# sigp/lighthouse

Hardware: AMD Instinct MI355X
Metric: bls_sig_sets_verified_per_sec (higher is better)
Workload: dtype u64; 1 GPU; c2_64k_attestation_sets_plus_c3_registry_root; n_sets_per_gpu=65536, set_mix=75% k=1 unagg, 25% aggregates k=512, n_validators=1048576, parallelism=single, full=False

## Files before the change

### include/m3x_consensus.h

```cpp
#ifndef M3X_CONSENSUS_H
#define M3X_CONSENSUS_H
#include <stdint.h>
#include <stddef.h>

#ifdef __cplusplus
extern "C" {
#endif

typedef struct m3x_ctx m3x_ctx;

#define M3X_OK 0
#define M3X_ERR_HIP -1
#define M3X_ERR_ARG -2
#define M3X_ERR_NOMEM -3
#define M3X_ERR_ENCODING -4

int32_t m3x_ctx_create(m3x_ctx **out, int32_t device);
void m3x_ctx_destroy(m3x_ctx *ctx);
int32_t m3x_abi_version(void);

int32_t m3x_timing_enable(m3x_ctx *ctx, int32_t on);
int32_t m3x_kernel_ms(m3x_ctx *ctx, int32_t kernel_id, double *ms,
                      uint64_t *launches);

// ... 6 lines not shown
int32_t m3x_h2d(m3x_ctx *ctx, void *dst_dev, const void *src_host,
                uint64_t bytes);
int32_t m3x_d2h(m3x_ctx *ctx, void *dst_host, const void *src_dev,
                uint64_t bytes);


int32_t m3x_merkleize_validators(m3x_ctx *ctx, const uint8_t *ssz, uint64_t n,
                                 uint8_t out_root[32]);
int32_t m3x_merkleize_validators_dev(m3x_ctx *ctx, const void *ssz_dev,
                                     uint64_t n, uint8_t out_root[32]);

int32_t m3x_merkleize_chunks(m3x_ctx *ctx, const uint8_t *chunks,
                             uint64_t n_chunks, uint32_t depth,
                             int64_t mix_len, uint8_t out_root[32]);
int32_t m3x_merkleize_chunks_dev(m3x_ctx *ctx, const void *chunks_dev,
                                 uint64_t n_chunks, uint32_t depth,
                                 int64_t mix_len, uint8_t out_root[32]);

int32_t m3x_validator_subtree_root_dev(m3x_ctx *ctx, const void *ssz_dev,
                                       uint64_t n, uint32_t depth,
                                       uint8_t out_root[32]);

typedef struct m3x_registry_cache m3x_registry_cache;

int32_t m3x_registry_cache_create(m3x_ctx *ctx, const uint8_t *ssz,
                                  uint64_t n, m3x_registry_cache **out);
void m3x_registry_cache_destroy(m3x_registry_cache *cache);
int32_t m3x_registry_cache_root(m3x_ctx *ctx, m3x_registry_cache *cache,
                                uint8_t out_root[32]);
int32_t m3x_registry_cache_update(m3x_ctx *ctx, m3x_registry_cache *cache,
                                  const uint64_t *indices,
                                  const uint8_t *recs , uint64_t m,
                                  uint8_t out_root[32]);

int32_t m3x_merkleize_batch(m3x_ctx *ctx, const uint8_t *chunks,
                            const uint32_t *offsets, uint64_t n_elems,
                            uint8_t *out_roots);

int32_t m3x_shuffle_list(m3x_ctx *ctx, uint32_t *indices, uint64_t list_size,
                         uint32_t rounds, const uint8_t seed[32],
                         int32_t forwards);
int32_t m3x_shuffle_list_dev(m3x_ctx *ctx, void *indices_dev,
                             uint64_t list_size, uint32_t rounds,
                             const uint8_t seed[32], int32_t forwards);


int32_t m3x_bls_expand_test(m3x_ctx *ctx, const uint8_t *msg,
                            uint32_t msg_len, const uint8_t *dst,
                            uint32_t dst_len, uint32_t len_in_bytes,
                            uint8_t *out);
int32_t m3x_bls_h2c_test(m3x_ctx *ctx, const uint8_t *msg, uint32_t msg_len,
                         const uint8_t *dst, uint32_t dst_len,
                         uint8_t out_uncomp[192], uint8_t out_uniform[256]);

int32_t m3x_bls_sig_sum_test(m3x_ctx *ctx, const uint8_t *sigs ,
                             const uint64_t *rands , uint64_t n,
                             int32_t use_msm, uint8_t out_uncomp[192]);

int32_t m3x_bls_pk_decompress(m3x_ctx *ctx, const uint8_t *comp ,
                              uint64_t n, uint8_t *uncomp ,
                              int32_t *status );

int32_t m3x_bls_sig_aggregate(m3x_ctx *ctx, const uint8_t *sigs ,
                              uint64_t n, uint8_t out_sig[96]);

int32_t m3x_bls_verify_sets(m3x_ctx *ctx, const uint8_t *msgs,
                            const uint8_t *sigs, const uint8_t *pks,
                            const uint32_t *pk_offsets, const uint64_t *rands,
                            uint64_t n);
int32_t m3x_bls_verify_sets_dev(m3x_ctx *ctx, const void *msgs_dev,
                                const void *sigs_dev, const void *pks_dev,
                                const void *pk_offsets_dev,
                                const void *rands_dev, uint64_t n);

int32_t m3x_bls_verify_each(m3x_ctx *ctx, const uint8_t *msgs,
                            const uint8_t *sigs, const uint8_t *pks,
                            const uint32_t *pk_offsets, uint64_t n,
                            int32_t *verdicts );
int32_t m3x_bls_verify_each_dev(m3x_ctx *ctx, const void *msgs_dev,
                                const void *sigs_dev, const void *pks_dev,
                                const void *pk_offsets_dev, uint64_t n,
                                void *verdicts_dev );

typedef struct m3x_kzg m3x_kzg;

int32_t m3x_kzg_create(m3x_ctx *ctx, const uint8_t g2_tau[96],
                       m3x_kzg **out);
void m3x_kzg_destroy(m3x_kzg *kzg);

int32_t m3x_kzg_verify_proof(m3x_ctx *ctx, m3x_kzg *kzg, const uint8_t c[48],
                             const uint8_t z[32], const uint8_t y[32],
                             const uint8_t proof[48]);
int32_t m3x_kzg_verify_proof_batch(m3x_ctx *ctx, m3x_kzg *kzg,
                                   const uint8_t *cs, const uint8_t *zs,
                                   const uint8_t *ys, const uint8_t *proofs,
                                   uint64_t n);
int32_t m3x_kzg_verify_blob_proof_batch(m3x_ctx *ctx, m3x_kzg *kzg,
                                        const uint8_t *blobs,
                                        const uint8_t *cs,
                                        const uint8_t *proofs, uint64_t n);
int32_t m3x_kzg_verify_blob_proof_batch_dev(m3x_ctx *ctx, m3x_kzg *kzg,
                                            const void *blobs_dev,
                                            const void *cs_dev,
                                            const void *proofs_dev,
                                            uint64_t n);

// ... 97 lines not shown
```

### lighthouse_amd/_native.py

```python
import ctypes
import os
import threading
from pathlib import Path

_PKG = Path(__file__).resolve().parent
_LIB_PATH = _PKG / "libm3x_consensus.so"

_lib = None
_load_error = None


def _bind(lib):
    lib.m3x_abi_version.restype = ctypes.c_int32
    lib.m3x_ctx_create.argtypes = [ctypes.POINTER(ctypes.c_void_p), ctypes.c_int32]
    lib.m3x_ctx_create.restype = ctypes.c_int32
    lib.m3x_ctx_destroy.argtypes = [ctypes.c_void_p]
    lib.m3x_dev_alloc.argtypes = [
        ctypes.c_void_p,
        ctypes.c_uint64,
        ctypes.POINTER(ctypes.c_void_p),
    ]
    lib.m3x_dev_alloc.restype = ctypes.c_int32
    lib.m3x_dev_free.argtypes = [ctypes.c_void_p, ctypes.c_void_p]
    lib.m3x_dev_free.restype = ctypes.c_int32
# ... 97 lines not shown
            ],
        ),
        (
            "m3x_merkleize_batch",
            [
                ctypes.c_void_p,
                ctypes.c_char_p,
                ctypes.POINTER(ctypes.c_uint32),
                ctypes.c_uint64,
                ctypes.c_char_p,
            ],
        ),
        (
            "m3x_kernel_ms",
            [
                ctypes.c_void_p,
                ctypes.c_int32,
                ctypes.POINTER(ctypes.c_double),
                ctypes.POINTER(ctypes.c_uint64),
            ],
        ),
        (
            "m3x_finalize_root",
            [
                ctypes.c_void_p,
                ctypes.c_char_p,
                ctypes.c_uint32,
                ctypes.c_uint32,
                ctypes.c_int64,
                ctypes.c_char_p,
            ],
        ),
        (
            "m3x_bls_expand_test",
            [
                ctypes.c_void_p,
                ctypes.c_char_p,
                ctypes.c_uint32,
                ctypes.c_char_p,
                ctypes.c_uint32,
                ctypes.c_uint32,
                ctypes.c_char_p,
            ],
        ),
        (
            "m3x_bls_h2c_test",
            [
                ctypes.c_void_p,
                ctypes.c_char_p,
                ctypes.c_uint32,
                ctypes.c_char_p,
                ctypes.c_uint32,
                ctypes.c_char_p,
                ctypes.c_char_p,
            ],
        ),
        (
            "m3x_bls_sig_sum_test",
            [
                ctypes.c_void_p,
                ctypes.c_char_p,
                ctypes.POINTER(ctypes.c_uint64),
                ctypes.c_uint64,
                ctypes.c_int32,
                ctypes.c_char_p,
            ],
        ),
        (
            "m3x_bls_pk_decompress",
            [
                ctypes.c_void_p,
                ctypes.c_char_p,
                ctypes.c_uint64,
                ctypes.c_char_p,
                ctypes.POINTER(ctypes.c_int32),
            ],
        ),
        (
            "m3x_bls_verify_sets",
            [
                ctypes.c_void_p,
                ctypes.c_char_p,
                ctypes.c_char_p,
                ctypes.c_char_p,
                ctypes.POINTER(ctypes.c_uint32),
                ctypes.POINTER(ctypes.c_uint64),
                ctypes.c_uint64,
            ],
        ),
        (
            "m3x_bls_verify_sets_dev",
            [
                ctypes.c_void_p,
                ctypes.c_void_p,
                ctypes.c_void_p,
                ctypes.c_void_p,
                ctypes.c_void_p,
                ctypes.c_void_p,
                ctypes.c_uint64,
            ],
        ),
        (
            "m3x_bls_verify_each",
            [
                ctypes.c_void_p,
                ctypes.c_char_p,
# ... 322 lines not shown
```

### lighthouse_amd/csrc/bls_device.hh

```
#pragma once
#include <hip/hip_runtime.h>
#include <stdint.h>
#include "bls_consts.h"
#include "sha256.hh"

namespace m3xb {

struct fp {
  uint64_t v[6];
};

struct fp2 {
  fp c0, c1;
};

struct g1a {
  fp x, y;
  int inf;
};
struct g1j {
  fp x, y, z;
};
struct g2a {
  fp2 x, y;
  int inf;
};
struct g2j {
  fp2 x, y, z;
};


__device__ __forceinline__ bool fp_ge_p(const uint64_t t[6]) {
#pragma unroll
  for (int i = 5; i >= 0; i--) {
    if (t[i] > BLS_P[i]) return true;
    if (t[i] < BLS_P[i]) return false;
  }
  return true;
}

__device__ __forceinline__ void fp_sub_p(uint64_t t[6]) {
  unsigned __int128 bw = 0;
#pragma unroll
  for (int i = 0; i < 6; i++) {
    unsigned __int128 x = (unsigned __int128)t[i] - BLS_P[i] - (uint64_t)bw;
    t[i] = (uint64_t)x;
    bw = (x >> 64) & 1;
  }
}

__device__ __forceinline__ void fp_add(fp &r, const fp &a, const fp &b) {
  unsigned __int128 c = 0;
  uint64_t t[6];
#pragma unroll
  for (int i = 0; i < 6; i++) {
    c += (unsigned __int128)a.v[i] + b.v[i];
// ... 180 lines not shown
__device__ __forceinline__ void fp_from_std(fp &r, const uint64_t std[6]) {
  fp s, r2;
#pragma unroll
  for (int i = 0; i < 6; i++) {
    s.v[i] = std[i];
    r2.v[i] = BLS_R2[i];
  }
  fp_mul(r, s, r2);
}

#define FP_LOAD_C(dst, NAME)                                                   \
  do {                                                                         \
    uint64_t _std[6] = {NAME[0], NAME[1], NAME[2], NAME[3], NAME[4], NAME[5]}; \
    fp_from_std(dst, _std);                                                    \
  } while (0)

__device__ __forceinline__ void fp_to_std(uint64_t std[6], const fp &a) {
  fp one_std;
#pragma unroll
  for (int i = 0; i < 6; i++) one_std.v[i] = (i == 0) ? 1ull : 0ull;
  fp t;
  fp_mul(t, a, one_std);
#pragma unroll
  for (int i = 0; i < 6; i++) std[i] = t.v[i];
}

__device__ inline void fp_pow_limbs(fp &r, const fp &a, const uint64_t *e,
                                    int n) {
  fp acc;
  fp_one(acc);
  bool started = false;
  for (int i = n - 1; i >= 0; i--) {
    for (int b = 63; b >= 0; b--) {
      if (started) fp_sqr(acc, acc);
      if ((e[i] >> b) & 1) {
        if (started)
          fp_mul(acc, acc, a);
        else {
          acc = a;
          started = true;
        }
      }
    }
  }
  r = acc;
}

__device__ inline void fp_inv(fp &r, const fp &a) {
  uint64_t e[6] = {BLS_P[0] - 2, BLS_P[1], BLS_P[2],
                   BLS_P[3], BLS_P[4], BLS_P[5]};
  fp_pow_limbs(r, a, e, 6);
}

__device__ inline bool fp_sqrt(fp &r, const fp &a) {
  uint64_t t[6] = {BLS_P[0] + 1, BLS_P[1], BLS_P[2],
                   BLS_P[3], BLS_P[4], BLS_P[5]};
  uint64_t e[6];
#pragma unroll
  for (int i = 0; i < 6; i++)
    e[i] = (t[i] >> 2) | (i < 5 ? (t[i + 1] << 62) : 0);
  fp s, s2;
  fp_pow_limbs(s, a, e, 6);
  fp_sqr(s2, s);
  if (!fp_eq(s2, a)) return false;
  r = s;
  return true;
}

__device__ inline bool fp_sqrt_ui(fp &s, fp &u, const fp &a) {
  uint64_t t[6] = {BLS_P[0] - 3, BLS_P[1], BLS_P[2],
                   BLS_P[3], BLS_P[4], BLS_P[5]};
  uint64_t e[6];
#pragma unroll
  for (int i = 0; i < 6; i++)
    e[i] = (t[i] >> 2) | (i < 5 ? (t[i + 1] << 62) : 0);
  fp_pow_limbs(u, a, e, 6);
  fp_mul(s, u, a);
  fp s2;
  fp_sqr(s2, s);
  return fp_eq(s2, a);
}

__device__ inline bool fp_gt_half(const fp &a) {
  uint64_t s[6];
  fp_to_std(s, a);
  uint64_t pm1[6] = {BLS_P[0] - 1, BLS_P[1], BLS_P[2],
                     BLS_P[3], BLS_P[4], BLS_P[5]};
  uint64_t h[6];
#pragma unroll
  for (int i = 0; i < 6; i++)
    h[i] = (pm1[i] >> 1) | (i < 5 ? (pm1[i + 1] << 63) : 0);
#pragma unroll
  for (int i = 5; i >= 0; i--) {
    if (s[i] > h[i]) return true;
    if (s[i] < h[i]) return false;
  }
  return false;
}

__device__ inline bool fp_is_odd_std(const fp &a) {
  uint64_t s[6];
  fp_to_std(s, a);
  return s[0] & 1;
}

__device__ inline bool fp_from_be48(fp &r, const uint8_t *b) {
  uint64_t s[6];
#pragma unroll
  for (int i = 0; i < 6; i++) {
    uint64_t w = 0;
#pragma unroll
    for (int j = 0; j < 8; j++) w = (w << 8) | b[8 * i + j];
    s[5 - i] = w;
  }
  if (fp_ge_p(s)) return false;
  fp_from_std(r, s);
  return true;
}

__device__ inline void fp_to_be48(const fp &a, uint8_t *b) {
  uint64_t s[6];
  fp_to_std(s, a);
#pragma unroll
  for (int i = 0; i < 6; i++)
#pragma unroll
    for (int j = 0; j < 8; j++)
      b[8 * i + j] = (uint8_t)(s[5 - i] >> (56 - 8 * j));
}

// ... 35 lines not shown
__device__ __forceinline__ void fp2_mul(fp2 &r, const fp2 &a, const fp2 &b) {
  fp t0, t1, s0, s1, m;
  fp_mul(t0, a.c0, b.c0);
  fp_mul(t1, a.c1, b.c1);
  fp_add(s0, a.c0, a.c1);
  fp_add(s1, b.c0, b.c1);
  fp_mul(m, s0, s1);
  fp_sub(m, m, t0);
  fp_sub(m, m, t1);
  fp_sub(r.c0, t0, t1);
  r.c1 = m;
}

__device__ __forceinline__ void fp2_sqr(fp2 &r, const fp2 &a) {
  fp s, d, m;
  fp_add(s, a.c0, a.c1);
  fp_sub(d, a.c0, a.c1);
  fp_mul(m, a.c0, a.c1);
  fp_mul(s, s, d);
  fp_add(r.c1, m, m);
  r.c0 = s;
}

__device__ __forceinline__ void fp2_mul_fp(fp2 &r, const fp2 &a, const fp &k) {
  fp_mul(r.c0, a.c0, k);
  fp_mul(r.c1, a.c1, k);
}

__device__ __forceinline__ void fp2_mul_small(fp2 &r, const fp2 &a, int k) {
  fp2 acc = a;
  for (int i = 1; i < k; i++) fp2_add(acc, acc, a);
  r = acc;
}

__device__ inline void fp2_inv(fp2 &r, const fp2 &a) {
  fp n, t0, t1;
  fp_sqr(t0, a.c0);
  fp_sqr(t1, a.c1);
  fp_add(n, t0, t1);
  fp_inv(n, n);
  fp_mul(r.c0, a.c0, n);
  fp_mul(t0, a.c1, n);
  fp_neg(r.c1, t0);
}

__device__ __forceinline__ void fp2_mul_xi(fp2 &r, const fp2 &a) {
  fp t0, t1;
  fp_sub(t0, a.c0, a.c1);
  fp_add(t1, a.c0, a.c1);
  r.c0 = t0;
  r.c1 = t1;
}

__device__ inline bool fp2_sqrt(fp2 &r, const fp2 &a) {
  if (fp2_is_zero(a)) {
    fp2_zero(r);
    return true;
  }
  if (fp_is_zero(a.c1)) {
    fp s;
    if (fp_sqrt(s, a.c0)) {
      r.c0 = s;
      fp_zero(r.c1);
      return true;
    }
    fp na;
    fp_neg(na, a.c0);
    if (!fp_sqrt(s, na)) return false;
    fp_zero(r.c0);
    r.c1 = s;
    return true;
  }
  fp n, s, d, x0, x1, t, u, inv2;
  fp_sqr(n, a.c0);
  fp_sqr(t, a.c1);
  fp_add(n, n, t);
  if (!fp_sqrt(s, n)) return false;
  FP_LOAD_C(inv2, FP_TWO_INV);
  fp_add(d, a.c0, s);
  fp_mul(d, d, inv2);
  if (!fp_sqrt_ui(x0, u, d)) {
    fp_sub(d, a.c0, s);
    fp_mul(d, d, inv2);
    if (!fp_sqrt_ui(x0, u, d)) return false;
  }
  fp_mul(x1, a.c1, u);
  fp_mul(x1, x1, inv2);
  fp2 cand, sq;
  cand.c0 = x0;
  cand.c1 = x1;
  fp2_sqr(sq, cand);
  if (!fp2_eq(sq, a)) return false;
  r = cand;
  return true;
}

__device__ inline bool fp2_gt_half_lex(const fp2 &y) {
  if (!fp_is_zero(y.c1)) return fp_gt_half(y.c1);
  if (!fp_is_zero(y.c0)) return fp_gt_half(y.c0);
  return false;
}

__device__ inline int fp2_sgn0(const fp2 &x) {
  int s0 = fp_is_odd_std(x.c0) ? 1 : 0;
  int z0 = fp_is_zero(x.c0) ? 1 : 0;
  int s1 = fp_is_odd_std(x.c1) ? 1 : 0;
  return s0 | (z0 & s1);
}

#define FP2_LOAD_C(dst, NAME)                                                  \
  do {                                                                         \
    FP_LOAD_C((dst).c0, NAME##_C0);                                            \
    FP_LOAD_C((dst).c1, NAME##_C1);                                            \
  } while (0)


__device__ __forceinline__ bool g1j_is_inf(const g1j &p) {
  return fp_is_zero(p.z);
}

__device__ __forceinline__ void g1j_set_inf(g1j &p) {
  fp_zero(p.x);
  fp_zero(p.y);
  fp_zero(p.z);
}

__device__ inline void g1j_from_aff(g1j &r, const g1a &a) {
  if (a.inf) {
    g1j_set_inf(r);
    return;
  }
  r.x = a.x;
  r.y = a.y;
  fp_one(r.z);
}

__device__ inline void g1j_to_aff(g1a &r, const g1j &p) {
  if (g1j_is_inf(p)) {
    r.inf = 1;
    fp_zero(r.x);
    fp_zero(r.y);
    return;
  }
// ... 1290 lines not shown
  for (int i = 0; i < dst_len; i++) cur[33 + i] = (uint8_t)DSTs[i];
  cur[33 + dst_len] = (uint8_t)dst_len;
  uint8_t bi[32];
  m3x::sha256_bytes(cur, 33 + dst_len + 1, bi);
  for (int i = 0; i < 32; i++) out[i] = bi[i];
  for (int blk = 2; blk <= 8; blk++) {
    for (int j = 0; j < 32; j++) cur[j] = b0[j] ^ bi[j];
    cur[32] = (uint8_t)blk;
    m3x::sha256_bytes(cur, 33 + dst_len + 1, bi);
    for (int j = 0; j < 32; j++) {
      bi[j] = bi[j];
      out[32 * (blk - 1) + j] = bi[j];
    }
  }
}

__device__ inline void expand_message_xmd_gen(const uint8_t *msg,
                                              uint32_t msg_len,
                                              const uint8_t *dst,
                                              uint32_t dst_len,
                                              uint32_t len_in_bytes,
                                              uint8_t *out) {
  uint32_t ell = (len_in_bytes + 31) / 32;
  uint8_t buf[64 + 544 + 2 + 1 + 255 + 1];
  uint32_t off = 0;
  for (int i = 0; i < 64; i++) buf[off++] = 0;
  for (uint32_t i = 0; i < msg_len; i++) buf[off++] = msg[i];
  buf[off++] = (uint8_t)(len_in_bytes >> 8);
  buf[off++] = (uint8_t)len_in_bytes;
  buf[off++] = 0;
  for (uint32_t i = 0; i < dst_len; i++) buf[off++] = dst[i];
  buf[off++] = (uint8_t)dst_len;
  uint8_t b0[32];
  m3x::sha256_bytes(buf, off, b0);
  uint8_t cur[32 + 1 + 255 + 1];
  for (int i = 0; i < 32; i++) cur[i] = b0[i];
  cur[32] = 1;
  for (uint32_t i = 0; i < dst_len; i++) cur[33 + i] = dst[i];
  cur[33 + dst_len] = (uint8_t)dst_len;
  uint8_t bi[32];
  m3x::sha256_bytes(cur, 33 + dst_len + 1, bi);
  uint32_t copied = len_in_bytes < 32 ? len_in_bytes : 32;
  for (uint32_t i = 0; i < copied; i++) out[i] = bi[i];
  for (uint32_t blk = 2; blk <= ell; blk++) {
    for (int j = 0; j < 32; j++) cur[j] = b0[j] ^ bi[j];
    cur[32] = (uint8_t)blk;
    m3x::sha256_bytes(cur, 33 + dst_len + 1, bi);
    uint32_t base = 32 * (blk - 1);
    uint32_t nc = len_in_bytes - base < 32 ? len_in_bytes - base : 32;
    for (uint32_t i = 0; i < nc; i++) out[base + i] = bi[i];
  }
}

__device__ inline void sswu_g2_tail(g2a &out, const fp2 &u, const fp2 &zu2,
                                    const fp2 &inv_tv_p1, bool tv_zero) {
  fp2 A, B;
  FP2_LOAD_C(A, SSWU_A);
  FP2_LOAD_C(B, SSWU_B);
  fp2 x1, gx1, y1, x, y, t;
  if (tv_zero) {
    FP2_LOAD_C(x1, SSWU_B_DIV_ZA);
  } else {
    fp2 nb_over_a;
    FP2_LOAD_C(nb_over_a, SSWU_NB_DIV_A);
    fp2_mul(x1, nb_over_a, inv_tv_p1);
  }
  fp2_sqr(gx1, x1);
  fp2_mul(gx1, gx1, x1);
  fp2_mul(t, A, x1);
  fp2_add(gx1, gx1, t);
  fp2_add(gx1, gx1, B);
  if (fp2_sqrt(y1, gx1)) {
    x = x1;
    y = y1;
  } else {
    fp2 x2, gx2;
    fp2_mul(x2, zu2, x1);
    fp2_sqr(gx2, x2);
    fp2_mul(gx2, gx2, x2);
    fp2_mul(t, A, x2);
    fp2_add(gx2, gx2, t);
    fp2_add(gx2, gx2, B);
    fp2_sqrt(y1, gx2);
    x = x2;
    y = y1;
  }
  if (fp2_sgn0(u) != fp2_sgn0(y)) fp2_neg(y, y);
  out.x = x;
  out.y = y;
  out.inf = 0;
}

__device__ inline void sswu_g2(g2a &out, const fp2 &u) {
  fp2 Z, zu2, tv, inv_tv;
  FP2_LOAD_C(Z, SSWU_Z);
  fp2_sqr(zu2, u);
  fp2_mul(zu2, zu2, Z);
  fp2_sqr(tv, zu2);
  fp2_add(tv, tv, zu2);
  bool tz = fp2_is_zero(tv);
  fp2_zero(inv_tv);
  if (!tz) {
    fp2 one;
    fp2_inv(inv_tv, tv);
    fp2_one(one);
    fp2_add(inv_tv, one, inv_tv);
  }
  sswu_g2_tail(out, u, zu2, inv_tv, tz);
}

__device__ inline void sswu_g2_dual(g2a out[2], const fp2 u[2]) {
  fp2 Z, zu2[2], tv[2];
  FP2_LOAD_C(Z, SSWU_Z);
  bool tz[2];
  for (int i = 0; i < 2; i++) {
    fp2_sqr(zu2[i], u[i]);
    fp2_mul(zu2[i], zu2[i], Z);
    fp2_sqr(tv[i], zu2[i]);
    fp2_add(tv[i], tv[i], zu2[i]);
    tz[i] = fp2_is_zero(tv[i]);
  }
  fp2 inv[2], one;
  fp2_one(one);
  if (!tz[0] && !tz[1]) {
    fp2 prod, pinv;
    fp2_mul(prod, tv[0], tv[1]);
    fp2_inv(pinv, prod);
    fp2_mul(inv[0], pinv, tv[1]);
    fp2_mul(inv[1], pinv, tv[0]);
  } else {
    for (int i = 0; i < 2; i++) {
      fp2_zero(inv[i]);
      if (!tz[i]) fp2_inv(inv[i], tv[i]);
    }
  }
  for (int i = 0; i < 2; i++) {
    fp2_add(inv[i], inv[i], one);
    sswu_g2_tail(out[i], u[i], zu2[i], inv[i], tz[i]);
  }
}

__device__ inline void iso_map_g2_j(g2j &out, const g2a &in) {
  fp2 k[4], xn, xd, yn, yd;
  FP2_LOAD_C(k[0], ISO_XNUM0);
  FP2_LOAD_C(k[1], ISO_XNUM1);
  FP2_LOAD_C(k[2], ISO_XNUM2);
  FP2_LOAD_C(k[3], ISO_XNUM3);
  xn = k[3];
  for (int i = 2; i >= 0; i--) {
    fp2_mul(xn, xn, in.x);
    fp2_add(xn, xn, k[i]);
  }
  FP2_LOAD_C(k[0], ISO_XDEN0);
  FP2_LOAD_C(k[1], ISO_XDEN1);
  FP2_LOAD_C(k[2], ISO_XDEN2);
  xd = k[2];
  for (int i = 1; i >= 0; i--) {
    fp2_mul(xd, xd, in.x);
    fp2_add(xd, xd, k[i]);
  }
  FP2_LOAD_C(k[0], ISO_YNUM0);
  FP2_LOAD_C(k[1], ISO_YNUM1);
  FP2_LOAD_C(k[2], ISO_YNUM2);
  FP2_LOAD_C(k[3], ISO_YNUM3);
  yn = k[3];
  for (int i = 2; i >= 0; i--) {
    fp2_mul(yn, yn, in.x);
    fp2_add(yn, yn, k[i]);
  }
  FP2_LOAD_C(k[0], ISO_YDEN0);
  FP2_LOAD_C(k[1], ISO_YDEN1);
  FP2_LOAD_C(k[2], ISO_YDEN2);
  FP2_LOAD_C(k[3], ISO_YDEN3);
  yd = k[3];
  for (int i = 2; i >= 0; i--) {
    fp2_mul(yd, yd, in.x);
    fp2_add(yd, yd, k[i]);
  }
  fp2 yd2, xd2, xd3, t;
  fp2_sqr(yd2, yd);
  fp2_sqr(xd2, xd);
  fp2_mul(xd3, xd2, xd);
  fp2_mul(out.z, xd, yd);
  fp2_mul(t, xn, xd);
  fp2_mul(out.x, t, yd2);
  fp2_mul(t, yd2, xd3);
  fp2_mul(t, t, yn);
  fp2_mul(out.y, t, in.y);
}

__device__ inline void g2j_neg(g2j &r, const g2j &p) {
  r.x = p.x;
// ... 1 lines not shown
  r.z = p.z;
}

__device__ inline void psi_g2j(g2j &r, const g2j &p) {
  fp2 cx, cy, t;
  FP2_LOAD_C(cx, PSI_CX);
  FP2_LOAD_C(cy, PSI_CY);
  fp2_conj(t, p.x);
  fp2_mul(r.x, t, cx);
  fp2_conj(t, p.y);
  fp2_mul(r.y, t, cy);
  fp2_conj(r.z, p.z);
}

__device__ inline void g2j_mul_u64_j(g2j &r, const g2j &base, uint64_t k) {
  g2j acc;
  g2j_set_inf(acc);
  for (int b = 63; b >= 0; b--) {
    g2j_dbl(acc, acc);
    if ((k >> b) & 1) g2j_add(acc, acc, base);
  }
  r = acc;
}

__device__ inline void clear_cofactor_g2j(g2j &out, const g2j &p) {
  g2j xp, xxp, acc, tmp, d;
  g2j_mul_u64_j(xp, p, BLS_X_ABS);
  g2j_neg(xp, xp);
  g2j_mul_u64_j(xxp, xp, BLS_X_ABS);
  g2j_neg(xxp, xxp);
  acc = xxp;
  g2j_neg(tmp, xp);
  g2j_add(acc, acc, tmp);
  g2j_neg(tmp, p);
  g2j_add(acc, acc, tmp);
  d = xp;
  g2j_neg(tmp, p);
  g2j_add(d, d, tmp);
  psi_g2j(tmp, d);
  g2j_add(acc, acc, tmp);
  g2j_dbl(tmp, p);
  psi_g2j(tmp, tmp);
  psi_g2j(tmp, tmp);
  g2j_add(acc, acc, tmp);
  out = acc;
}

__device__ inline void h2c_g2_from_uniform(g2j &r, const uint8_t uni[256]) {
  fp2 u[2];
  h2f_from_be64(u[0].c0, uni);
  h2f_from_be64(u[0].c1, uni + 64);
  h2f_from_be64(u[1].c0, uni + 128);
  h2f_from_be64(u[1].c1, uni + 192);
  g2a qp[2];
  sswu_g2_dual(qp, u);
  g2j s, t;
  iso_map_g2_j(s, qp[0]);
  iso_map_g2_j(t, qp[1]);
  g2j_add(s, s, t);
  clear_cofactor_g2j(r, s);
}

__device__ inline void h2c_g2(g2j &r, const uint8_t *msg) {
  uint8_t uni[256];
  expand_message_xmd32(msg, uni);
  h2c_g2_from_uniform(r, uni);
}

__device__ inline void g2_to_uncomp_dev(const g2a &p, uint8_t *out) {
  fp_to_be48(p.x.c1, out);
  fp_to_be48(p.x.c0, out + 48);
  fp_to_be48(p.y.c1, out + 96);
  fp_to_be48(p.y.c0, out + 144);
}

__device__ inline void g1_gen(g1a &g) {
  FP_LOAD_C(g.x, BLS_G1X);
  FP_LOAD_C(g.y, BLS_G1Y);
  g.inf = 0;
}


template <typename T, int W, typename Op>
__device__ __forceinline__ void block_tree_reduce(T *lds, int t, Op op) {
  __syncthreads();
  for (int s = W / 2; s > 0; s >>= 1) {
    if (t < s) {
      T r;
      op(r, lds[t], lds[t + s]);
      lds[t] = r;
    }
    __syncthreads();
  }
}

struct g1j_add_op {
  __device__ __forceinline__ void operator()(g1j &r, const g1j &a,
                                             const g1j &b) const {
    g1j_add(r, a, b);
  }
};
struct g2j_add_op {
  __device__ __forceinline__ void operator()(g2j &r, const g2j &a,
                                             const g2j &b) const {
    g2j_add(r, a, b);
  }
};

template <typename T, int W, typename Op, typename Ident>
__device__ __forceinline__ void block_span_reduce(const T *__restrict__ in,
                                                  uint64_t n,
                                                  T *__restrict__ out, T *lds,
// ... 19 lines not shown
```

### lighthouse_amd/csrc/m3x_bls.hip

```cpp
#include "bls_device.hh"
#include "m3x_ctx.hh"
#include "../../include/m3x_consensus.h"
#include <cstdio>
#include <cstdlib>

static bool dbg_sync() {
  static int v = -1;
  if (v < 0) {
    const char *e = getenv("M3X_DEBUG_SYNC");
    v = (e && e[0] == '1') ? 1 : 0;
  }
  return v == 1;
}
#define DBG_STEP(ctx, name)                                                    \
  do {                                                                         \
    if (dbg_sync()) {                                                          \
      hipError_t _e = hipStreamSynchronize((ctx)->stream);                     \
      fprintf(stderr, "[m3x dbg] %s: %s\n", name, hipGetErrorString(_e));      \
      fflush(stderr);                                                          \
    }                                                                          \
  } while (0)

using namespace m3xb;

// ... 350 lines not shown
    }
    if (!sg.inf) {
      g2j sj;
      g2j_from_aff(sj, sg);
      g2j_add(acc, acc, sj);
    }
  }
  if (bad) atomicOr(fail, 1);
  lds[lane] = acc;
  block_tree_reduce<g2j, 64>(lds, lane, g2j_add_op{});
  if (lane == 0 && !*fail) {
    g2a a;
    g2j_to_aff(a, lds[0]);
    if (a.inf) {
      for (int i = 0; i < 96; i++) out[i] = 0;
      out[0] = 0xC0;
    } else {
      fp_to_be48(a.x.c1, out);
      fp_to_be48(a.x.c0, out + 48);
      out[0] |= 0x80;
      if (fp2_gt_half_lex(a.y)) out[0] |= 0x20;
    }
  }
}

__global__ void k_bls_h2c_dst(const uint8_t *__restrict__ msg,
                              uint32_t msg_len,
                              const uint8_t *__restrict__ dst,
                              uint32_t dst_len, uint8_t *__restrict__ out,
                              uint8_t *__restrict__ uni_out) {
  if (blockIdx.x != 0 || threadIdx.x != 0) return;
  uint8_t uni[256];
  expand_message_xmd_gen(msg, msg_len, dst, dst_len, 256, uni);
  for (int i = 0; i < 256; i++) uni_out[i] = uni[i];
  g2j h;
  h2c_g2_from_uniform(h, uni);
  g2a a;
  g2j_to_aff(a, h);
  g2_to_uncomp_dev(a, out);
}

__global__ void k_bls_g2j_uncomp(const g2j *__restrict__ p,
                                 uint8_t *__restrict__ out,
                                 int32_t *__restrict__ is_inf) {
  if (blockIdx.x != 0 || threadIdx.x != 0) return;
  g2a a;
  g2j_to_aff(a, p[0]);
  *is_inf = a.inf ? 1 : 0;
  if (a.inf) {
    for (int i = 0; i < 192; i++) out[i] = 0;
    return;
  }
  g2_to_uncomp_dev(a, out);
}

__global__ void k_bls_expand_dst(const uint8_t *__restrict__ msg,
                                 uint32_t msg_len,
                                 const uint8_t *__restrict__ dst,
                                 uint32_t dst_len, uint32_t len_in_bytes,
                                 uint8_t *__restrict__ out) {
  if (blockIdx.x != 0 || threadIdx.x != 0) return;
  expand_message_xmd_gen(msg, msg_len, dst, dst_len, len_in_bytes, out);
}

template <typename Fail>
__device__ __forceinline__ void sigdec_lane(const uint8_t *__restrict__ sigs,
                                            uint64_t n, const BlsWork &w,
                                            Fail fail) {
  uint64_t i = (uint64_t)blockIdx.x * blockDim.x + threadIdx.x;
  if (i >= n) return;
  g2a sig;
  if (g2_decompress(sig, sigs + 96 * i) != 0) {
    fail.mark(i);
    sig.inf = 1;
  }
  g2j out;
  g2j_from_aff(out, sig);
  w.sig_aff[i] = out;
}

__global__ __launch_bounds__(64) __attribute__((amdgpu_waves_per_eu(1, 1)))
void k_bls_sigdec_lat(const uint8_t *__restrict__ sigs, uint64_t n,
                      BlsWork w) {
  sigdec_lane(sigs, n, w, BatchFail{w.fail});
}

__global__ __launch_bounds__(64) __attribute__((amdgpu_waves_per_eu(1, 1)))
void k_bls_sigdec_each(const uint8_t *__restrict__ sigs, uint64_t n,
                       BlsWork w, int32_t *__restrict__ status) {
  sigdec_lane(sigs, n, w, SetFail{status});
}

template <int First, int Last>
__device__ __forceinline__ void prep_mults_lane(
    const uint8_t *__restrict__ pks, const uint32_t *__restrict__ offs,
    const uint64_t *__restrict__ rands, uint64_t n, const BlsWork &w) {
  uint64_t lane = (uint64_t)blockIdx.x * blockDim.x + threadIdx.x;
  if (lane >= (uint64_t)(Last - First + 1) * n) return;
  int cls = First + (lane < n ? 0 : (lane < 2 * n ? 1 : 2));
  uint64_t i = lane - (uint64_t)(cls - First) * n;
  if (First == 0 && cls == 0) {
    g2a sig;
    sig_aff_load(sig, w.sig_aff[i]);
    if (sig.inf) {
      g2j_set_inf(w.rsig[i]);
      return;
// ... 345 lines not shown
  M3X_HIP_CHECK(hipSetDevice(ctx->device));
  m3x::DevTemps tmp(ctx->stream);
  const uint8_t *comp_d = tmp.upload(comp, n * 48);
  uint8_t *unc_d = tmp.alloc(n * 96);
  int32_t *st_d = tmp.alloc<int32_t>(n * 4);
  if (!tmp.ok()) return M3X_ERR_HIP;
  uint32_t blocks = (uint32_t)((n + 63) / 64);
  hipLaunchKernelGGL(k_bls_pk_decompress, dim3(blocks), dim3(64), 0,
                     ctx->stream, comp_d, n, unc_d, st_d);
  tmp.download(uncomp, unc_d, n * 96);
  tmp.download(status, st_d, n * 4);
  return tmp.sync() ? M3X_OK : M3X_ERR_HIP;
}

int32_t m3x_bls_expand_test(m3x_ctx *ctx, const uint8_t *msg,
                            uint32_t msg_len, const uint8_t *dst,
                            uint32_t dst_len, uint32_t len_in_bytes,
                            uint8_t *out) {
  if (!ctx || msg_len > 544 || dst_len == 0 || dst_len > 255 ||
      len_in_bytes > 256)
    return M3X_ERR_ARG;
  std::lock_guard<std::recursive_mutex> lk(ctx->mu);
  M3X_HIP_CHECK(hipSetDevice(ctx->device));
  m3x::DevTemps tmp(ctx->stream);
  const uint8_t *msg_d = tmp.upload(msg, msg_len);
  const uint8_t *dst_d = tmp.upload(dst, dst_len);
  uint8_t *out_d = tmp.alloc(256);
  if (!tmp.ok()) return M3X_ERR_HIP;
  hipLaunchKernelGGL(k_bls_expand_dst, dim3(1), dim3(1), 0, ctx->stream,
                     msg_d, msg_len, dst_d, dst_len, len_in_bytes, out_d);
  tmp.download(out, out_d, len_in_bytes);
  return tmp.sync() ? M3X_OK : M3X_ERR_HIP;
}

int32_t m3x_bls_h2c_test(m3x_ctx *ctx, const uint8_t *msg, uint32_t msg_len,
                         const uint8_t *dst, uint32_t dst_len,
                         uint8_t out_uncomp[192], uint8_t out_uniform[256]) {
  if (!ctx || msg_len > 544 || dst_len == 0 || dst_len > 255)
    return M3X_ERR_ARG;
  std::lock_guard<std::recursive_mutex> lk(ctx->mu);
  M3X_HIP_CHECK(hipSetDevice(ctx->device));
  m3x::DevTemps tmp(ctx->stream);
  const uint8_t *msg_d = tmp.upload(msg, msg_len);
  const uint8_t *dst_d = tmp.upload(dst, dst_len);
  uint8_t *pt_d = tmp.alloc(192), *uni_d = tmp.alloc(256);
  if (!tmp.ok()) return M3X_ERR_HIP;
  hipLaunchKernelGGL(k_bls_h2c_dst, dim3(1), dim3(1), 0, ctx->stream, msg_d,
                     msg_len, dst_d, dst_len, pt_d, uni_d);
  tmp.download(out_uncomp, pt_d, 192);
  if (out_uniform) tmp.download(out_uniform, uni_d, 256);
  return tmp.sync() ? M3X_OK : M3X_ERR_HIP;
}

int32_t m3x_bls_sig_sum_test(m3x_ctx *ctx, const uint8_t *sigs,
                             const uint64_t *rands, uint64_t n,
                             int32_t use_msm, uint8_t out_uncomp[192]) {
  if (!ctx || !sigs || !rands || !out_uncomp || n == 0 ||
      n > m3x::kSigMsmMaxSets)
    return M3X_ERR_ARG;
  std::lock_guard<std::recursive_mutex> lk(ctx->mu);
  M3X_HIP_CHECK(hipSetDevice(ctx->device));
  BlsWork w = {};
  int32_t *is_inf = nullptr;
  uint8_t *out_d = nullptr;
  int rc = m3x::carve_scratch(
      ctx, &ctx->scratch_a, &ctx->scratch_a_bytes, [&](m3x::ScratchCarver &c) {
        w.rsig = c.take<g2j>(n);
        w.sig_aff = c.take<g2j>(n);
        w.fail = c.take<int>(1);
        w.sig_stage = c.take<g2j>(kReduceMaxBlocks);
        w.sig_sum = c.take<g2j>(1);
        is_inf = c.take<int32_t>(1);
        out_d = c.take<uint8_t>(192);
        carve_sig_msm(c, w, n);
      });
  if (rc != M3X_OK) return rc;
  m3x::DevTemps tmp(ctx->stream);
  const uint8_t *sigs_d = tmp.upload(sigs, n * 96);
  const uint64_t *rands_d = tmp.upload(rands, n * 8);
  if (!tmp.ok()) return M3X_ERR_HIP;
  M3X_HIP_CHECK(hipMemsetAsync(w.fail, 0, 4, ctx->stream));
  uint32_t blocks = (uint32_t)((n + 63) / 64);
  hipLaunchKernelGGL(k_bls_sigdec_lat, dim3(blocks), dim3(64), 0, ctx->stream,
                     sigs_d, n, w);
  if (use_msm) {
    rc = m3x::launch_bls_sig_msm(ctx->stream, n, w.sig_aff, rands_d, w.msm,
                                 w.sig_sum);
    if (rc != M3X_OK) {
      (void)tmp.sync();
      return rc;
    }
  } else {
    hipLaunchKernelGGL(k_bls_prep_rsig, dim3(blocks), dim3(64), 0, ctx->stream,
                       rands_d, n, w);
    uint32_t sblocks = (uint32_t)((n + kReduceThreads - 1) / kReduceThreads);
    if (sblocks > kReduceMaxBlocks) sblocks = kReduceMaxBlocks;
    hipLaunchKernelGGL(k_bls_reduce_sig, dim3(sblocks), dim3(kReduceThreads),
                       0, ctx->stream, w.rsig, n, w.sig_stage);
    hipLaunchKernelGGL(k_bls_reduce_sig, dim3(1), dim3(kReduceThreads), 0,
                       ctx->stream, w.sig_stage, (uint64_t)sblocks, w.sig_sum);
  }
  hipLaunchKernelGGL(k_bls_g2j_uncomp, dim3(1), dim3(1), 0, ctx->stream,
                     w.sig_sum, out_d, is_inf);
  int32_t fail = 1, inf = 0;
  tmp.download(out_uncomp, out_d, 192);
  tmp.download(&fail, w.fail, 4);
// ... 97 lines not shown
```

Baseline: 649,900 sets/s.

## Replace SSWU G2 map with single-exponentiation norm-based fast path

Rewrites the simplified SWU map to G2 so it uses a projective x = xn/xd form. The fp2 square root and the inversion come from one Fp exponentiation of a norm, with selects instead of branches, so the separate fp2 inversion and multiple sqrt attempts are no longer needed. Degenerate cases fall back to a noinline slow path. The dual batched inversion over two field elements is dropped in favour of a per-element loop. Test entry points are added for sqrt, SSWU and batch hash-to-curve. The risk is correctness on edge cases and higher register pressure in the fast path.

```diff
diff --git a/include/m3x_consensus.h b/include/m3x_consensus.h
--- a/include/m3x_consensus.h
+++ b/include/m3x_consensus.h
@@ -82,6 +82,17 @@
 int32_t m3x_bls_h2c_test(m3x_ctx *ctx, const uint8_t *msg, uint32_t msg_len,
                          const uint8_t *dst, uint32_t dst_len,
                          uint8_t out_uncomp[192], uint8_t out_uniform[256]);
+
+int32_t m3x_bls_fp2_sqrt_test(m3x_ctx *ctx, const uint8_t *a ,
+                              uint64_t n, uint8_t *out ,
+                              uint8_t *ok );
+int32_t m3x_bls_sswu_test(m3x_ctx *ctx, const uint8_t *u ,
+                          uint64_t n, uint8_t *out );
+int32_t m3x_bls_sswu_slow_test(m3x_ctx *ctx, const uint8_t *u ,
+                               uint64_t n, uint8_t *out );
+int32_t m3x_bls_h2c_batch_test(m3x_ctx *ctx, const uint8_t *msgs ,
+                               uint64_t n, int32_t mode,
+                               uint8_t *out );
 
 int32_t m3x_bls_sig_sum_test(m3x_ctx *ctx, const uint8_t *sigs ,
                              const uint64_t *rands , uint64_t n,
diff --git a/lighthouse_amd/_native.py b/lighthouse_amd/_native.py
--- a/lighthouse_amd/_native.py
+++ b/lighthouse_amd/_native.py
@@ -173,6 +173,34 @@
                 ctypes.c_char_p,
                 ctypes.c_uint32,
                 ctypes.c_char_p,
+                ctypes.c_char_p,
+            ],
+        ),
+        (
+            "m3x_bls_fp2_sqrt_test",
+            [
+                ctypes.c_void_p,
+                ctypes.c_char_p,
+                ctypes.c_uint64,
+                ctypes.c_char_p,
+                ctypes.c_char_p,
+            ],
+        ),
+        (
+            "m3x_bls_sswu_test",
+            [ctypes.c_void_p, ctypes.c_char_p, ctypes.c_uint64, ctypes.c_char_p],
+        ),
+        (
+            "m3x_bls_sswu_slow_test",
+            [ctypes.c_void_p, ctypes.c_char_p, ctypes.c_uint64, ctypes.c_char_p],
+        ),
+        (
+            "m3x_bls_h2c_batch_test",
+            [
+                ctypes.c_void_p,
+                ctypes.c_char_p,
+                ctypes.c_uint64,
+                ctypes.c_int32,
                 ctypes.c_char_p,
             ],
         ),
diff --git a/lighthouse_amd/csrc/bls_device.hh b/lighthouse_amd/csrc/bls_device.hh
--- a/lighthouse_amd/csrc/bls_device.hh
+++ b/lighthouse_amd/csrc/bls_device.hh
@@ -2,6 +2,7 @@
 #include <hip/hip_runtime.h>
 #include <stdint.h>
 #include "bls_consts.h"
+#include "bls_h2c_consts.h"
 #include "sha256.hh"
 
 namespace m3xb {
@@ -288,15 +289,34 @@
   fp_pow_limbs(r, a, e, 6);
 }
 
-__device__ inline bool fp_sqrt(fp &r, const fp &a) {
+__device__ __forceinline__ void fp_sel(fp &r, bool c, const fp &a,
+                                       const fp &b) {
+#pragma unroll
+  for (int i = 0; i < 6; i++) r.v[i] = c ? a.v[i] : b.v[i];
+}
+
+__device__ inline void fp_pow_m3(fp &r, const fp &a) {
+  uint64_t t[6] = {BLS_P[0] - 3, BLS_P[1], BLS_P[2],
+                   BLS_P[3], BLS_P[4], BLS_P[5]};
+  uint64_t e[6];
+#pragma unroll
+  for (int i = 0; i < 6; i++)
+    e[i] = (t[i] >> 2) | (i < 5 ? (t[i + 1] << 62) : 0);
+  fp_pow_limbs(r, a, e, 6);
+}
+__device__ inline void fp_pow_p1(fp &r, const fp &a) {
   uint64_t t[6] = {BLS_P[0] + 1, BLS_P[1], BLS_P[2],
                    BLS_P[3], BLS_P[4], BLS_P[5]};
   uint64_t e[6];
 #pragma unroll
   for (int i = 0; i < 6; i++)
     e[i] = (t[i] >> 2) | (i < 5 ? (t[i + 1] << 62) : 0);
+  fp_pow_limbs(r, a, e, 6);
+}
+
+__device__ inline bool fp_sqrt(fp &r, const fp &a) {
   fp s, s2;
-  fp_pow_limbs(s, a, e, 6);
+  fp_pow_p1(s, a);
   fp_sqr(s2, s);
   if (!fp_eq(s2, a)) return false;
   r = s;
@@ -304,13 +324,7 @@
 }
 
 __device__ inline bool fp_sqrt_ui(fp &s, fp &u, const fp &a) {
-  uint64_t t[6] = {BLS_P[0] - 3, BLS_P[1], BLS_P[2],
-                   BLS_P[3], BLS_P[4], BLS_P[5]};
-  uint64_t e[6];
-#pragma unroll
-  for (int i = 0; i < 6; i++)
-    e[i] = (t[i] >> 2) | (i < 5 ? (t[i + 1] << 62) : 0);
-  fp_pow_limbs(u, a, e, 6);
+  fp_pow_m3(u, a);
   fp_mul(s, u, a);
   fp s2;
   fp_sqr(s2, s);
@@ -452,6 +466,36 @@
   r.c1 = t1;
 }
 
+__device__ __forceinline__ void fp2_sel(fp2 &r, bool c, const fp2 &a,
+                                        const fp2 &b) {
+  fp_sel(r.c0, c, a.c0, b.c0);
+  fp_sel(r.c1, c, a.c1, b.c1);
+}
+
+__device__ __forceinline__ void fp2_norm(fp &n, const fp2 &a) {
+  fp t;
+  fp_sqr(n, a.c0);
+  fp_sqr(t, a.c1);
+  fp_add(n, n, t);
+}
+
+__device__ inline void fp2_sqrt_from_norm_root(fp2 &r, const fp2 &a,
+                                               const fp &s) {
+  fp inv2, d, u, t, h, nh, t2;
+  FP_LOAD_C(inv2, FP_TWO_INV);
+  fp_add(d, a.c0, s);
+  fp_mul(d, d, inv2);
+  fp_pow_m3(u, d);
+  fp_mul(t, u, d);
+  fp_mul(h, a.c1, u);
+  fp_mul(h, h, inv2);
+  fp_neg(nh, h);
+  fp_sqr(t2, t);
+  bool plus = fp_eq(t2, d);
+  fp_sel(r.c0, plus, t, nh);
+  fp_sel(r.c1, plus, h, t);
+}
+
 __device__ inline bool fp2_sqrt(fp2 &r, const fp2 &a) {
   if (fp2_is_zero(a)) {
     fp2_zero(r);
@@ -471,24 +515,11 @@
     r.c1 = s;
     return true;
   }
-  fp n, s, d, x0, x1, t, u, inv2;
-  fp_sqr(n, a.c0);
-  fp_sqr(t, a.c1);
-  fp_add(n, n, t);
+  fp n, s;
+  fp2_norm(n, a);
   if (!fp_sqrt(s, n)) return false;
-  FP_LOAD_C(inv2, FP_TWO_INV);
-  fp_add(d, a.c0, s);
-  fp_mul(d, d, inv2);
-  if (!fp_sqrt_ui(x0, u, d)) {
-    fp_sub(d, a.c0, s);
-    fp_mul(d, d, inv2);
-    if (!fp_sqrt_ui(x0, u, d)) return false;
-  }
-  fp_mul(x1, a.c1, u);
-  fp_mul(x1, x1, inv2);
   fp2 cand, sq;
-  cand.c0 = x0;
-  cand.c1 = x1;
+  fp2_sqrt_from_norm_root(cand, a, s);
   fp2_sqr(sq, cand);
   if (!fp2_eq(sq, a)) return false;
   r = cand;
@@ -1885,92 +1916,122 @@
   }
 }
 
-__device__ inline void sswu_g2_tail(g2a &out, const fp2 &u, const fp2 &zu2,
-                                    const fp2 &inv_tv_p1, bool tv_zero) {
-  fp2 A, B;
+__device__ __noinline__ void sswu_g2_slow(g2a &out, const fp2 &u) {
+  fp2 A, B, Z, zu2, tv, x1, gx, y, t;
   FP2_LOAD_C(A, SSWU_A);
   FP2_LOAD_C(B, SSWU_B);
-  fp2 x1, gx1, y1, x, y, t;
-  if (tv_zero) {
-    FP2_LOAD_C(x1, SSWU_B_DIV_ZA);
-  } else {
-    fp2 nb_over_a;
-    FP2_LOAD_C(nb_over_a, SSWU_NB_DIV_A);
-    fp2_mul(x1, nb_over_a, inv_tv_p1);
-  }
-  fp2_sqr(gx1, x1);
-  fp2_mul(gx1, gx1, x1);
-  fp2_mul(t, A, x1);
-  fp2_add(gx1, gx1, t);
-  fp2_add(gx1, gx1, B);
-  if (fp2_sqrt(y1, gx1)) {
-    x = x1;
-    y = y1;
-  } else {
-    fp2 x2, gx2;
-    fp2_mul(x2, zu2, x1);
-    fp2_sqr(gx2, x2);
-    fp2_mul(gx2, gx2, x2);
-    fp2_mul(t, A, x2);
-    fp2_add(gx2, gx2, t);
-    fp2_add(gx2, gx2, B);
-    fp2_sqrt(y1, gx2);
-    x = x2;
-    y = y1;
-  }
-  if (fp2_sgn0(u) != fp2_sgn0(y)) fp2_neg(y, y);
-  out.x = x;
-  out.y = y;
-  out.inf = 0;
-}
-
-__device__ inline void sswu_g2(g2a &out, const fp2 &u) {
-  fp2 Z, zu2, tv, inv_tv;
   FP2_LOAD_C(Z, SSWU_Z);
   fp2_sqr(zu2, u);
   fp2_mul(zu2, zu2, Z);
   fp2_sqr(tv, zu2);
   fp2_add(tv, tv, zu2);
-  bool tz = fp2_is_zero(tv);
-  fp2_zero(inv_tv);
-  if (!tz) {
-    fp2 one;
-    fp2_inv(inv_tv, tv);
+  if (fp2_is_zero(tv)) {
+    FP2_LOAD_C(x1, SSWU_B_DIV_ZA);
+  } else {
+    fp2 nb_over_a, one;
+    FP2_LOAD_C(nb_over_a, SSWU_NB_DIV_A);
+    fp2_inv(t, tv);
     fp2_one(one);
-    fp2_add(inv_tv, one, inv_tv);
-  }
-  sswu_g2_tail(out, u, zu2, inv_tv, tz);
-}
-
-__device__ inline void sswu_g2_dual(g2a out[2], const fp2 u[2]) {
-  fp2 Z, zu2[2], tv[2];
+    fp2_add(t, t, one);
+    fp2_mul(x1, nb_over_a, t);
+  }
+#pragma unroll 1
+  for (int c = 0; c < 2; c++) {
+    fp2_sqr(gx, x1);
+    fp2_add(gx, gx, A);
+    fp2_mul(gx, gx, x1);
+    fp2_add(gx, gx, B);
+    if (fp2_sqrt(y, gx)) break;
+    fp2_mul(x1, zu2, x1);
+  }
+  if (fp2_sgn0(u) != fp2_sgn0(y)) fp2_neg(y, y);
+  out.x = x1;
+  out.y = y;
+  out.inf = 0;
+}
+
+__device__ __noinline__ bool sswu_g2_fast(g2a &out, const fp2 &u) {
+  fp2 A, B, Z, zu2, tv, xn, xd, a, t;
+  fp ng, nzu, n;
+  FP2_LOAD_C(A, SSWU_A);
+  FP2_LOAD_C(B, SSWU_B);
   FP2_LOAD_C(Z, SSWU_Z);
-  bool tz[2];
-  for (int i = 0; i < 2; i++) {
-    fp2_sqr(zu2[i], u[i]);
-    fp2_mul(zu2[i], zu2[i], Z);
-    fp2_sqr(tv[i], zu2[i]);
-    fp2_add(tv[i], tv[i], zu2[i]);
-    tz[i] = fp2_is_zero(tv[i]);
-  }
-  fp2 inv[2], one;
-  fp2_one(one);
-  if (!tz[0] && !tz[1]) {
-    fp2 prod, pinv;
-    fp2_mul(prod, tv[0], tv[1]);
-    fp2_inv(pinv, prod);
-    fp2_mul(inv[0], pinv, tv[1]);
-    fp2_mul(inv[1], pinv, tv[0]);
-  } else {
-    for (int i = 0; i < 2; i++) {
-      fp2_zero(inv[i]);
-      if (!tz[i]) fp2_inv(inv[i], tv[i]);
-    }
-  }
-  for (int i = 0; i < 2; i++) {
-    fp2_add(inv[i], inv[i], one);
-    sswu_g2_tail(out[i], u[i], zu2[i], inv[i], tz[i]);
-  }
+  fp2_sqr(zu2, u);
+  fp2_mul(zu2, zu2, Z);
+  fp2_sqr(tv, zu2);
+  fp2_add(tv, tv, zu2);
+  {
+    fp2 one, za, xd2, gn;
+    fp2_one(one);
+    fp2_add(xn, tv, one);
+    fp2_mul(xn, xn, B);
+    fp2_mul(xd, A, tv);
+    fp2_neg(xd, xd);
+    fp2_mul(za, Z, A);
+    fp2_sel(xd, fp2_is_zero(tv), za, xd);
+    fp2_sqr(xd2, xd);
+    fp2_sqr(gn, xn);
+    fp2_mul(t, A, xd2);
+    fp2_add(gn, gn, t);
+    fp2_mul(gn, gn, xn);
+    fp2_mul(t, xd2, xd);
+    fp2_mul(t, t, B);
+    fp2_add(gn, gn, t);
+    fp2_mul(a, gn, xd);
+    fp2_norm(ng, gn);
+    fp nu;
+    fp2_norm(nzu, zu2);
+    fp2_norm(nu, u);
+    fp_mul(nzu, nzu, nu);
+  }
+  fp2_norm(n, a);
+  fp u1, s1, chk;
+  fp_pow_m3(u1, n);
+  fp_mul(s1, u1, n);
+  fp_sqr(chk, s1);
+  bool is_sq = fp_eq(chk, n);
+  fp2 sel;
+  fp s;
+  {
+    fp2 a2;
+    fp c5, s2;
+    fp2_sqr(t, zu2);
+    fp2_mul(t, t, zu2);
+    fp2_mul(a2, t, a);
+    FP_LOAD_C(c5, FP_SQRT_NEG5);
+    fp_mul(s2, nzu, c5);
+    fp_mul(s2, s2, s1);
+    fp2_sel(sel, is_sq, a, a2);
+    fp_sel(s, is_sq, s1, s2);
+  }
+  if (fp_is_zero(n) || fp_is_zero(sel.c1)) return false;
+  fp2 x, xdi2;
+  {
+    fp ninv, nn, k;
+    fp2 xdi, xz;
+    fp_sqr(ninv, u1);
+    fp_neg(nn, ninv);
+    fp_sel(ninv, is_sq, ninv, nn);
+    fp_mul(k, ng, ninv);
+    fp2_conj(xdi, xd);
+    fp2_mul_fp(xdi, xdi, k);
+    fp2_mul(x, xn, xdi);
+    fp2_mul(xz, x, zu2);
+    fp2_sel(x, is_sq, x, xz);
+    fp2_sqr(xdi2, xdi);
+  }
+  fp2 root, y;
+  fp2_sqrt_from_norm_root(root, sel, s);
+  fp2_mul(y, root, xdi2);
+  if (fp2_sgn0(u) != fp2_sgn0(y)) fp2_neg(y, y);
+  out.x = x;
+  out.y = y;
+  out.inf = 0;
+  return true;
+}
+
+__device__ __forceinline__ void sswu_g2(g2a &out, const fp2 &u) {
+  if (!sswu_g2_fast(out, u)) sswu_g2_slow(out, u);
 }
 
 __device__ inline void iso_map_g2_j(g2j &out, const g2a &in) {
@@ -2078,12 +2139,15 @@
   h2f_from_be64(u[0].c1, uni + 64);
   h2f_from_be64(u[1].c0, uni + 128);
   h2f_from_be64(u[1].c1, uni + 192);
-  g2a qp[2];
-  sswu_g2_dual(qp, u);
-  g2j s, t;
-  iso_map_g2_j(s, qp[0]);
-  iso_map_g2_j(t, qp[1]);
-  g2j_add(s, s, t);
+  g2j pt[2];
+#pragma unroll 1
+  for (int i = 0; i < 2; i++) {
+    g2a q;
+    sswu_g2(q, u[i]);
+    iso_map_g2_j(pt[i], q);
+  }
+  g2j s;
+  g2j_add(s, pt[0], pt[1]);
   clear_cofactor_g2j(r, s);
 }
 
diff --git a/lighthouse_amd/csrc/bls_h2c_consts.h b/lighthouse_amd/csrc/bls_h2c_consts.h
--- /dev/null
+++ b/lighthouse_amd/csrc/bls_h2c_consts.h
@@ -0,0 +1,5 @@
+#ifndef M3X_BLS_H2C_CONSTS_H
+#define M3X_BLS_H2C_CONSTS_H
+#include "bls_consts.h"
+static M3X_CONST uint64_t FP_SQRT_NEG5[6] = {0x4d39c9db7b263cd4ULL, 0x6c12a6d436befcf9ULL, 0xa014c40bceb7d230ULL, 0x4614aa5e2eebdeb1ULL, 0x7a88b0f999ab2b50ULL, 0x186417302d5a6534ULL};
+#endif
diff --git a/lighthouse_amd/csrc/m3x_bls.hip b/lighthouse_amd/csrc/m3x_bls.hip
--- a/lighthouse_amd/csrc/m3x_bls.hip
+++ b/lighthouse_amd/csrc/m3x_bls.hip
@@ -426,6 +426,60 @@
     return;
   }
   g2_to_uncomp_dev(a, out);
+}
+
+__global__ __launch_bounds__(64) void k_bls_fp2_sqrt_test(
+    const uint8_t *__restrict__ in, uint64_t n, uint8_t *__restrict__ out,
+    uint8_t *__restrict__ ok) {
+  uint64_t i = (uint64_t)blockIdx.x * blockDim.x + threadIdx.x;
+  if (i >= n) return;
+  fp2 a, r;
+  fp2_zero(r);
+  bool good = fp_from_be48(a.c0, in + 96 * i) &&
+              fp_from_be48(a.c1, in + 96 * i + 48);
+  if (good) good = fp2_sqrt(r, a);
+  if (!good) fp2_zero(r);
+  fp_to_be48(r.c0, out + 96 * i);
+  fp_to_be48(r.c1, out + 96 * i + 48);
+  ok[i] = good ? 1 : 0;
+}
+
+__global__ __launch_bounds__(64) void k_bls_sswu_test(
+    const uint8_t *__restrict__ in, uint64_t n, int slow,
+    uint8_t *__restrict__ out) {
+  uint64_t i = (uint64_t)blockIdx.x * blockDim.x + threadIdx.x;
+  if (i >= n) return;
+  fp2 u;
+  g2a q, a;
+  a.inf = 1;
+  if (fp_from_be48(u.c0, in + 96 * i) &&
+      fp_from_be48(u.c1, in + 96 * i + 48)) {
+    g2j pt;
+    if (slow)
+      sswu_g2_slow(q, u);
+    else
+      sswu_g2(q, u);
+    iso_map_g2_j(pt, q);
+    g2j_to_aff(a, pt);
+  }
+  if (a.inf) {
+    for (int b = 0; b < 192; b++) out[192 * i + b] = 0;
+    return;
+  }
+  g2_to_uncomp_dev(a, out + 192 * i);
+}
+
+__global__ __launch_bounds__(64) void k_bls_h2c_uncomp_test(
+    uint64_t n, BlsWork w, uint8_t *__restrict__ out) {
+  uint64_t i = (uint64_t)blockIdx.x * blockDim.x + threadIdx.x;
+  if (i >= n) return;
+  g2a a;
+  g2j_to_aff(a, w.h2c[i]);
+  if (a.inf) {
+    for (int b = 0; b < 192; b++) out[192 * i + b] = 0;
+    return;
+  }
+  g2_to_uncomp_dev(a, out + 192 * i);
 }
 
 __global__ void k_bls_expand_dst(const uint8_t *__restrict__ msg,
@@ -877,6 +931,96 @@
   return tmp.sync() ? M3X_OK : M3X_ERR_HIP;
 }
 
+int32_t m3x_bls_fp2_sqrt_test(m3x_ctx *ctx, const uint8_t *a, uint64_t n,
+                              uint8_t *out, uint8_t *ok) {
+  if (!ctx || !a || !out || !ok || n == 0 || n > (1u << 20))
+    return M3X_ERR_ARG;
+  std::lock_guard<std::recursive_mutex> lk(ctx->mu);
+  M3X_HIP_CHECK(hipSetDevice(ctx->device));
+  m3x::DevTemps tmp(ctx->stream);
+  const uint8_t *a_d = tmp.upload(a, n * 96);
+  uint8_t *out_d = tmp.alloc(n * 96), *ok_d = tmp.alloc(n);
+  if (!tmp.ok()) return M3X_ERR_HIP;
+  uint32_t blocks = (uint32_t)((n + 63) / 64);
+  hipLaunchKernelGGL(k_bls_fp2_sqrt_test, dim3(blocks), dim3(64), 0,
+                     ctx->stream, a_d, n, out_d, ok_d);
+  tmp.download(out, out_d, n * 96);
+  tmp.download(ok, ok_d, n);
+  return tmp.sync() ? M3X_OK : M3X_ERR_HIP;
+}
+
+static int32_t sswu_test(m3x_ctx *ctx, const uint8_t *u, uint64_t n, int slow,
+                         uint8_t *out) {
+  if (!ctx || !u || !out || n == 0 || n > (1u << 20)) return M3X_ERR_ARG;
+  std::lock_guard<std::recursive_mutex> lk(ctx->mu);
+  M3X_HIP_CHECK(hipSetDevice(ctx->device));
+  m3x::DevTemps tmp(ctx->stream);
+  const uint8_t *u_d = tmp.upload(u, n * 96);
+  uint8_t *out_d = tmp.alloc(n * 192);
+  if (!tmp.ok()) return M3X_ERR_HIP;
+  uint32_t blocks = (uint32_t)((n + 63) / 64);
+  hipLaunchKernelGGL(k_bls_sswu_test, dim3(blocks), dim3(64), 0, ctx->stream,
+                     u_d, n, slow, out_d);
+  tmp.download(out, out_d, n * 192);
+  return tmp.sync() ? M3X_OK : M3X_ERR_HIP;
+}
+
+int32_t m3x_bls_sswu_test(m3x_ctx *ctx, const uint8_t *u, uint64_t n,
+                          uint8_t *out) {
+  return sswu_test(ctx, u, n, 0, out);
+}
+
+int32_t m3x_bls_sswu_slow_test(m3x_ctx *ctx, const uint8_t *u, uint64_t n,
+                               uint8_t *out) {
+  return sswu_test(ctx, u, n, 1, out);
+}
+
+int32_t m3x_bls_h2c_batch_test(m3x_ctx *ctx, const uint8_t *msgs, uint64_t n,
+                               int32_t mode, uint8_t *out) {
+  if (!ctx || !msgs || !out || n == 0 || n > (1u << 20) || mode < 0 ||
+      mode > 2)
+    return M3X_ERR_ARG;
+  std::lock_guard<std::recursive_mutex> lk(ctx->mu);
+  M3X_HIP_CHECK(hipSetDevice(ctx->device));
+  BlsWork w = {};
+  uint8_t *out_d = nullptr;
+  int rc = m3x::carve_scratch(
+      ctx, &ctx->scratch_a, &ctx->scratch_a_bytes, [&](m3x::ScratchCarver &c) {
+        w.h2c = c.take<g2j>(n);
+        w.uni = c.take<uint8_t>(n * 256);
+        w.h2c_pts = c.take<g2j>(2 * n);
+        out_d = c.take<uint8_t>(n * 192);
+      });
+  if (rc != M3X_OK) return rc;
+  m3x::DevTemps tmp(ctx->stream);
+  const uint8_t *msgs_d = tmp.upload(msgs, n * 32);
+  if (!tmp.ok()) return M3X_ERR_HIP;
+  uint32_t blocks = (uint32_t)((n + 63) / 64);
+  uint32_t blocks2 = (uint32_t)((2 * n + 63) / 64);
+  if (mode == 0) {
+    hipLaunchKernelGGL(k_bls_h2c, dim3(blocks), dim3(64), 0, ctx->stream,
+                       msgs_d, n, w);
+  } else {
+    hipLaunchKernelGGL(k_bls_h2c_expand, dim3(blocks), dim3(64), 0,
+                       ctx->stream, msgs_d, n, w);
+    if (mode == 1) {
+      hipLaunchKernelGGL(k_bls_h2c_map, dim3(blocks2), dim3(64), 0,
+                         ctx->stream, n, w);
+      hipLaunchKernelGGL(k_bls_h2c_fin, dim3(blocks), dim3(64), 0,
+                         ctx->stream, n, w);
+    } else {
+      hipLaunchKernelGGL(k_bls_h2c_map_lat, dim3(blocks2), dim3(64), 0,
+                         ctx->stream, n, w);
+      hipLaunchKernelGGL(k_bls_h2c_fin_lat, dim3(blocks), dim3(64), 0,
+                         ctx->stream, n, w);
+    }
+  }
+  hipLaunchKernelGGL(k_bls_h2c_uncomp_test, dim3(blocks), dim3(64), 0,
+                     ctx->stream, n, w, out_d);
+  tmp.download(out, out_d, n * 192);
+  return tmp.sync() ? M3X_OK : M3X_ERR_HIP;
+}
+
 int32_t m3x_bls_sig_sum_test(m3x_ctx *ctx, const uint8_t *sigs,
                              const uint64_t *rands, uint64_t n,
                              int32_t use_msm, uint8_t out_uncomp[192]) {
```

Measured after the change: 709,800 sets/s (median of 6 runs). +9.2%, better.
